# stanfordnlp/mac-network

Measured on AMD Instinct MI355X. Metric: questions/sec fwd+bwd (B=64,d=512,p=12,KB=14x14x1024) at 1/2/4/8 MI355X, higher is better.
Workload: dtype f32 (3xfp16-split emulation); 1 GPU

## Files before the change

include/macx.h:

```cpp
#ifndef MACX_H
#define MACX_H

#include <stddef.h>
#include <stdint.h>

#ifdef __cplusplus
extern "C" {
#endif

#define MACX_ABI_VERSION 5

enum {
  MACX_OK = 0,
  MACX_EINVAL = -1,
  MACX_EUNSUPPORTED = -2,
  MACX_EREJECTED = -3,
  MACX_ESMALL = -4,
  MACX_EWAIT = -5
};

enum { MACX_ACT_NON = 0, MACX_ACT_TANH = 1, MACX_ACT_SIGMOID = 2, MACX_ACT_ELU = 3, MACX_ACT_RELU = 4 };
enum { MACX_INIT_PRM = 0, MACX_INIT_ZERO = 1, MACX_INIT_Q = 2 };
enum { MACX_WRITE_MEM = 0, MACX_WRITE_INFO = 1, MACX_WRITE_SUM = 2, MACX_WRITE_BOTH = 3 };

// ... 241 lines not shown
                       const float* d_kb, const macx_stem_grads*, void* stream);
int macx_stem_forward_w(const macx_stem_shapes*, int act, float keep, uint32_t seed, const macx_stem_params*,
                        const float* images, float* kb, float* saved, size_t saved_floats, const uint32_t* mask_word, void* stream);
int macx_stem_backward_w(const macx_stem_shapes*, int act, float keep, uint32_t seed, const macx_stem_params*,
                         const float* kb, const float* saved, size_t saved_floats, float* ws, size_t ws_floats,
                         const float* d_kb, const macx_stem_grads*, const uint32_t* mask_word, void* stream);

typedef struct macx_conv_shapes { int32_t B, H, W, Cin, Cout, k, stride; } macx_conv_shapes;
size_t macx_conv2d_ws_floats(const macx_conv_shapes*);
int macx_conv2d_fwd(const macx_conv_shapes*, const float* x, const float* w, const float* bias, float* y, void* stream);
int macx_conv2d_bwd_data(const macx_conv_shapes*, const float* dy, const float* w, float* dx, void* stream);
int macx_conv2d_wgrad(const macx_conv_shapes*, const float* x, const float* dy, float* dw, float* ws, size_t ws_floats,
                      void* stream);

int macx_images_to_nhwc(const float* nchw, int B, int C, int HW, float* nhwc, void* stream);

typedef struct macx_enc_shapes { int32_t B, S, V, E, h, b0; } macx_enc_shapes;
typedef struct macx_enc_params { const float* emb; const float* fw_kernel; const float* fw_bias; const float* bw_kernel; const float* bw_bias; } macx_enc_params;
typedef struct macx_enc_grads { float* emb; float* fw_kernel; float* fw_bias; float* bw_kernel; float* bw_bias; } macx_enc_grads;
size_t macx_encoder_saved_floats(const macx_enc_shapes*);
size_t macx_encoder_ws_floats(const macx_enc_shapes*);
int macx_encoder_forward(const macx_enc_shapes*, float keep_input, float keep_question, uint32_t seed, const macx_enc_params*,
                         const int32_t* questions , const int32_t* lengths , float* words ,
                         float* vecQuestions , float* saved, size_t saved_floats, void* stream);
int macx_encoder_backward(const macx_enc_shapes*, float keep_input, float keep_question, uint32_t seed, const macx_enc_params*,
                          const int32_t* questions, const int32_t* lengths, const float* saved, size_t saved_floats,
                          float* ws, size_t ws_floats, const float* d_words, const float* d_vecQuestions,
                          const macx_enc_grads*, void* stream);
int macx_encoder_forward_w(const macx_enc_shapes*, float keep_input, float keep_question, uint32_t seed, const macx_enc_params*,
                           const int32_t* questions , const int32_t* lengths , float* words ,
                           float* vecQuestions , float* saved, size_t saved_floats, const uint32_t* mask_word,
                           void* stream);
int macx_encoder_backward_w(const macx_enc_shapes*, float keep_input, float keep_question, uint32_t seed, const macx_enc_params*,
                            const int32_t* questions, const int32_t* lengths, const float* saved, size_t saved_floats,
                            float* ws, size_t ws_floats, const float* d_words, const float* d_vecQuestions,
                            const macx_enc_grads*, const uint32_t* mask_word, void* stream);

int macx_adam_ema_step(size_t n, float* params, const float* grads, float* m, float* v, float* ema,
                       float lr, float beta1, float beta2, float eps, int step, float clip_norm, float ema_decay,
                       float* ws, float* norm_out, void* stream);
int macx_adam_ema_step_p(size_t n, float* params, const float* grads, float* m, float* v, float* ema,
                         const float* lr_t_dev, float beta1, float beta2, float eps, float clip_norm, float ema_decay,
                         float* ws, float* norm_out, void* stream);
int macx_adam_ema_step_g(size_t n, float* params, const float* grads, float* m, float* v, float* ema,
                         float lr, float beta1, float beta2, float eps, int step, float clip_norm, float ema_decay,
                         float skip_above, uint32_t* guard, float* ws, float* norm_out, void* stream);
int macx_adam_ema_step_pg(size_t n, float* params, const float* grads, float* m, float* v, float* ema,
                          const float* lr_t_dev, float beta1, float beta2, float eps, float clip_norm, float ema_decay,
                          float skip_above, uint32_t* guard, float* ws, float* norm_out, void* stream);

typedef struct macx_gather_entry { const float* src; uint64_t dst_offset; uint64_t count; } macx_gather_entry;
int macx_gather_flat(const macx_gather_entry* table_dev, int entries, float* flat, void* stream);

int macx_kb_gather(const float* kb_images , const int32_t* image_index , int G, int B, int N, int d,
                   float* kb , void* stream);
int macx_kb_gather_bwd(const float* dkb , const int32_t* image_index , int G, int B, int N, int d,
                       float* dkb_images , void* stream);
int macx_kb_gather_l(const float* kb_images , const int32_t* image_index ,
                     const int32_t* image_lengths , int G, int B, int N, int d, float* kb ,
                     int32_t* kb_lengths_out , void* stream);
int macx_kb_gather_bwd_l(const float* dkb , const int32_t* image_index ,
                         const int32_t* image_lengths , int G, int B, int N, int d,
                         float* dkb_images , void* stream);

enum { MACX_FEATURES_F32 = 0, MACX_FEATURES_F16 = 1 };
int macx_features_pack(const float* src, int layout, int n, int C, int HW, void* table, int dtype, size_t row0, size_t rows,
                       int32_t* overflow , void* stream);
int macx_features_gather(const void* table, int dtype, size_t rows, const int32_t* ids , int G, int C, int HW,
                         float* out , void* stream);

int macx_questions_gather(const int32_t* q_words , const int32_t* q_lengths , const int32_t* q_answers ,
                          const int32_t* q_images , const int32_t* q_kb_len ,
                          const float* q_weights , int Q, int S_tab, const int32_t* ids , int B,
                          int S , int32_t* questions , int32_t* lengths , int32_t* answers ,
                          int32_t* image_ids , int32_t* kb_lengths ,
                          float* weights , int32_t* image_index , int G,
                          int32_t* bad , void* stream);
int macx_preds_scatter(const int32_t* pred , const int32_t* ids , int B, int Q, int32_t* table ,
                       void* stream);

int macx_linear(const float* x1, int k1, const float* x2, int k2, int rows,
                const float* W_packed, const float* b, float bias_const, int n_out, int act,
                float* out, void* stream);
#define MACX_PACK_TRANSPOSE 1
#define MACX_PACK_F32MFMA (0 << 1)
#define MACX_PACK_BF16X3 (1 << 1)
#define MACX_PACK_KMAJOR (2 << 1)
int macx_pack_weight(const float* W, int K, int n_out, int flags, float* out, void* stream);
#define MACX_GEMM_NATIVE 0
#define MACX_GEMM_SPLIT 1
#define MACX_GEMM_H2 2
int macx_gemm_mode(int mode);

size_t macx_h2_floats(size_t rows, size_t cols);
int macx_h2_from_f32(const float* src, int B, int N, int C, float* h2, void* stream);
int macx_h2_to_f32(const float* h2, int rows, int C, float* out, void* stream);
int macx_h2_pack_weight(const float* W, int K, int n_out, int transpose, float* out, void* stream);
int macx_h2_gemm_planes(const float* hA, int B, int N, int K, const float* Wh, int n_out, const float* bias, int act, float* hO,
                        void* stream);
int macx_h2_gemm(const float* A, int B, int N, int K, const float* W, int n_out, const float* bias, int act, float* out,
                 float* ws, size_t ws_floats, void* stream);
size_t macx_h2_wgrad_ws_floats(const macx_opts* o, int nt, int R, int Kd, int Jd, int nsplit, int pair);
int macx_h2_wgrad(const macx_opts* o, int nt, int R, int Kd, int Jd, int nsplit, const float* hA, size_t a_stride, int a_shared,
                  const float* hG, size_t g_stride, float* out, const float* hA2, size_t a2_stride, int a2_shared, const float* hG2,
                  size_t g2_stride, float* out2, float* ws, size_t ws_floats, void* stream);
size_t macx_h2_sb_ws_floats(const macx_opts* o, int B, int N, int d, int nsteps, int qpg, int wide);
int macx_h2_sb(const macx_opts* o, int B, int N, int d, int nsteps, int qpg, int wide, const float* hX, size_t x_stride,
               const float* hdI1, size_t g_stride, const float* y, const float* W1a, float* dW1a, float* dW1b, float* dy_part,
               float* ws, size_t ws_floats, void* stream);
int macx_read_chain_time(const macx_opts*, const macx_shapes*, const macx_dropout*, const macx_params*, const macx_inputs*,
                         float* saved, size_t saved_floats, int step, int reps, float* ms_out, void* stream);
int macx_cell_forward_chain_time(const macx_opts*, const macx_shapes*, const macx_dropout*, const macx_params*, const macx_inputs*,
                                 float* saved, size_t saved_floats, float* ws, size_t ws_floats, float* ms_out, void* stream);
int macx_saved_activation(const macx_opts*, const macx_shapes*, int which, int step, const float* saved, size_t saved_floats,
                          float* out, void* stream);
size_t macx_ctrl_inputs_ws_floats(const macx_opts*, const macx_shapes*);
int macx_ctrl_inputs_fwd(const macx_opts*, const macx_shapes*, const macx_params*, const float* vecQuestions, float* ctrl_t,
                         float* ctrl_inputs, float* ws, size_t ws_floats, void* stream);
int macx_ctrl_inputs_bwd(const macx_opts*, const macx_shapes*, const macx_params*, const float* vecQuestions, const float* ctrl_t,
                         const float* d_ctrl_inputs, const macx_param_grads*, float* d_vecQuestions, float* ws, size_t ws_floats,
                         void* stream);
int macx_kb_project(const macx_shapes*, const macx_dropout*, int step, const float* kb,
                    const float* W_packed, const float* b, float* out, float* drop_ws, void* stream);
int macx_control_attend(const macx_shapes*, const float* cc, const float* words, const int32_t* lengths,
                        const float* w, const float* b, float* att, float* control, void* stream);
size_t macx_control_attend_bwd_ws_floats(const macx_shapes*);
int macx_control_attend_bwd(const macx_shapes*, const float* d_control, const float* cc, const float* att, const float* words,
                            const float* w, float* ws, size_t ws_floats, float* d_cc, float* d_words, float* d_w, float* d_b,
                            void* stream);
int macx_dropout_mask(uint32_t seed, uint32_t site, uint32_t step, float keep, uint32_t first,
                      size_t n, float* out, void* stream);
int macx_dropout_mask_w(uint32_t seed, uint32_t site, uint32_t step, float keep, uint32_t first,
                        size_t n, const uint32_t* mask_word, float* out, void* stream);
int macx_wgrad_splits(int M, int Kd, int Jd);
int macx_wgrad(const float* A, int lda, const float* G, int ldg, int M, int Kd, int Jd,
               float* out, float* ws, void* stream);

int macx_answer_loss(const float* logits, const int32_t* answers, int B, int A, float* loss_rows, int32_t* pred,
                     float* dlogits, float grad_scale, void* stream);

enum { MACX_ATT_LOSS_CE = 0, MACX_ATT_LOSS_ENTROPY = 1 };
int macx_att_loss(const float* att, const float* target, const int32_t* lengths, const float* step_weights,
                  const float* row_weights, int p, int B, int n, int kind, int target_steps, float eps, float scale,
                  float* loss_rows, float* d_att, void* stream);

int macx_answer_loss_weighted(const float* logits, const int32_t* answers, const float* weights, int B, int A,
                              float* loss_rows, int32_t* pred, float* dlogits, float* loss_out, double* totals,
                              float grad_scale, void* stream);

int macx_kb_attend_fwd(int B, int N, int d, const float* logits, const float* bias, const float* kb, float* att, float* info,
                       void* stream);
int macx_kb_attend_fwd_l(int B, int N, int d, const float* logits, const float* bias, const float* kb, const int32_t* kb_lengths,
                         float* att, float* info, void* stream);
size_t macx_kb_attend_bwd_ws_floats(int B, int N, int d);
int macx_kb_attend_bwd(int B, int N, int d, const float* att, const float* kb, const float* dinfo, float* dlogits, float* dkb,
                       int accumulate, float* ws, size_t ws_floats, void* stream);

size_t macx_workspace_bytes(const macx_opts*, const macx_shapes*, int for_backward);
int macx_read_fwd(const macx_opts*, const macx_shapes*, const macx_dropout*, const macx_params*, const float* knowledgeBase,
                  const float* memory, const float* control, float* saved, size_t saved_floats, float* info, float* att,
                  void* stream);
int macx_read_fwd_l(const macx_opts*, const macx_shapes*, const macx_dropout*, const macx_params*, const float* knowledgeBase,
                    const int32_t* kb_lengths, const float* memory, const float* control, float* saved, size_t saved_floats,
                    float* info, float* att, void* stream);
int macx_read_bwd(const macx_opts*, const macx_shapes*, const macx_dropout*, const macx_params*, const float* knowledgeBase,
                  const float* saved, size_t saved_floats, float* ws, size_t ws_floats, const float* d_info,
// ... 39 lines not shown
```

mac-network_amd/_lib.py:

```python
import ctypes as C
import os

import torch

from . import build as _build

ABI_VERSION = 5

MACX_OK, MACX_EINVAL, MACX_EUNSUPPORTED, MACX_EREJECTED, MACX_ESMALL, MACX_EWAIT = 0, -1, -2, -3, -4, -5
HANDOFF_BITS = {1: "a chain tile gave up waiting for its step's y", 2: "a filler workgroup gave up waiting for the previous step's write unit"}
STATUS_WORDS = 16
ACT = {"NON": 0, "TANH": 1, "SIGMOID": 2, "ELU": 3, "RELU": 4}
INIT = {"PRM": 0, "ZERO": 1, "Q": 2}
WRITE_INPUTS = {"MEM": 0, "INFO": 1, "SUM": 2, "BOTH": 3}
SEG = {"controls": 0, "memories": 1, "infos": 2, "att_question": 3, "att_kb": 4, "att_self": 5, "att_gate": 6,
       "status": 7}


class MacxOpts(C.Structure):
    _fields_ = [(n, C.c_int32) for n in (
        "abi_version", "init_ctrl", "init_mem", "control_input_unshared", "control_input_act", "control_feed_prev",
        "control_feed_prev_att", "control_feed_inputs", "control_cont_act", "read_mem_act", "read_ctrl_act",
        "write_inputs", "write_self_att", "write_self_att_cont", "write_mem_act", "write_gate", "write_gate_shared")]
    _fields_ += [("write_gate_bias", C.c_float), ("memory_variational_dropout", C.c_int32), ("gemm_family", C.c_int32),
# ... 115 lines not shown
_I, _U, _Z, _F, _V = C.c_int, C.c_uint32, C.c_size_t, C.c_float, C.c_void_p


def _masked(sig):
    restype, a = sig
    return restype, a[:-1] + (_V, a[-1])


_OS = (_P(MacxOpts), _P(MacxShapes))
_RUN = _OS + (_P(MacxDropout), _P(MacxParams), _P(MacxInputs), _V, _Z, _V, _Z)
_BWD = _RUN + (_V, _V, _P(MacxParamGrads), _P(MacxInputGrads))
_UNIT = _OS + (_P(MacxDropout), _P(MacxParams))
_STEM = (_P(MacxStemShapes), _I, _F, _U, _P(MacxStemParams))
_OUT = (_P(MacxOutShapes), _I, _F, _U, _P(MacxOutParams))
_ENC = (_P(MacxEncShapes), _F, _F, _U, _P(MacxEncParams))
_GATHER = (_V, _V, _I, _I, _I, _I, _V, _V)

TABLE = {}
TABLE.update(
    macx_saved_floats=(_Z, _OS + (_I,)),
    macx_ws_floats=(_Z, _OS + (_I,)),
    macx_saved_segment=(_I, _OS + (_I, _I, _P(_Z), _P(_Z))),
    macx_check=(_I, _OS),
    macx_cell_route=(_I, _OS + (_P(MacxDropout), _I, _I, _P(MacxRoute))))
TABLE.update(
    macx_run_status=(_I, _OS + (_I, _V, _Z, _V, _P(_U), _P(C.c_int32))),
    macx_run_status_reset=(_I, _OS + (_I, _V, _Z, _V)),
    macx_handoff_selftest=(_I, (_V, _P(_U))))
TABLE.update(
    macx_cell_begin=(_I, _RUN + (_I, _V)),
    macx_cell_step=(_I, _RUN + (_I, _I, _V)),
    macx_cell_forward=(_I, _RUN + (_I, _V)),
    macx_cell_backward=(_I, _BWD + (_V,)),
    macx_cell_backward_phase=(_I, _BWD + (_I, _V)),
    macx_cell_backward_x=(_I, _BWD + (_P(MacxStateGrads), _V)),
    macx_cell_backward_phase_x=(_I, _BWD + (_P(MacxStateGrads), _I, _V)))
TABLE.update(
    macx_output_saved_floats=(_Z, (_P(MacxOutShapes),)),
    macx_output_ws_floats=(_Z, (_P(MacxOutShapes),)),
    macx_output_forward=(_I, _OUT + (_V, _V, _V, _V, _Z, _V)),
    macx_output_backward=(_I, _OUT + (_V, _V, _V, _Z, _V, _Z, _V, _P(MacxOutGrads), _V, _V, _V)))
TABLE.update(macx_output_forward_w=_masked(TABLE["macx_output_forward"]),
             macx_output_backward_w=_masked(TABLE["macx_output_backward"]))
TABLE.update(
    macx_stem_saved_floats=(_Z, (_P(MacxStemShapes),)),
    macx_stem_ws_floats=(_Z, (_P(MacxStemShapes),)),
    macx_stem_forward=(_I, _STEM + (_V, _V, _V, _Z, _V)),
    macx_stem_backward=(_I, _STEM + (_V, _V, _Z, _V, _Z, _V, _P(MacxStemGrads), _V)))
TABLE.update(macx_stem_forward_w=_masked(TABLE["macx_stem_forward"]),
             macx_stem_backward_w=_masked(TABLE["macx_stem_backward"]))
TABLE.update(
    macx_conv2d_ws_floats=(_Z, (_P(MacxConvShapes),)),
    macx_conv2d_fwd=(_I, (_P(MacxConvShapes), _V, _V, _V, _V, _V)),
    macx_conv2d_bwd_data=(_I, (_P(MacxConvShapes), _V, _V, _V, _V)),
    macx_conv2d_wgrad=(_I, (_P(MacxConvShapes), _V, _V, _V, _V, _Z, _V)),
    macx_images_to_nhwc=(_I, (_V, _I, _I, _I, _V, _V)))
TABLE.update(
    macx_encoder_saved_floats=(_Z, (_P(MacxEncShapes),)),
    macx_encoder_ws_floats=(_Z, (_P(MacxEncShapes),)),
    macx_encoder_forward=(_I, _ENC + (_V, _V, _V, _V, _V, _Z, _V)),
    macx_encoder_backward=(_I, _ENC + (_V, _V, _V, _Z, _V, _Z, _V, _V, _P(MacxEncGrads), _V)))
TABLE.update(macx_encoder_forward_w=_masked(TABLE["macx_encoder_forward"]),
             macx_encoder_backward_w=_masked(TABLE["macx_encoder_backward"]))
TABLE.update(
    macx_adam_ema_step=(_I, (_Z, _V, _V, _V, _V, _V, _F, _F, _F, _F, _I, _F, _F, _V, _V, _V)),
    macx_adam_ema_step_p=(_I, (_Z, _V, _V, _V, _V, _V, _V, _F, _F, _F, _F, _F, _V, _V, _V)),
    macx_adam_ema_step_g=(_I, (_Z, _V, _V, _V, _V, _V, _F, _F, _F, _F, _I, _F, _F, _F, _V, _V, _V, _V)),
    macx_adam_ema_step_pg=(_I, (_Z, _V, _V, _V, _V, _V, _V, _F, _F, _F, _F, _F, _F, _V, _V, _V, _V)))
TABLE.update(macx_gather_flat=(_I, (_V, _I, _V, _V)))
TABLE.update(
    macx_kb_gather=(_I, _GATHER),
    macx_kb_gather_bwd=(_I, _GATHER),
    macx_kb_gather_l=(_I, _GATHER[:2] + (_V,) + _GATHER[2:-1] + (_V, _GATHER[-1])),
    macx_kb_gather_bwd_l=(_I, _GATHER[:2] + (_V,) + _GATHER[2:]))
TABLE.update(
    macx_features_pack=(_I, (_V, _I, _I, _I, _I, _V, _I, _Z, _Z, _V, _V)),
    macx_features_gather=(_I, (_V, _I, _Z, _V, _I, _I, _I, _V, _V)))
FEATURES_DTYPE = {torch.float32: 0, torch.float16: 1}
TABLE.update(
    macx_questions_gather=(_I, (_V,) * 6 + (_I, _I, _V, _I, _I) + (_V,) * 6 + (_V, _I, _V, _V)),
    macx_preds_scatter=(_I, (_V, _V, _I, _I, _V, _V)))
TABLE.update(
    macx_linear=(_I, (_V, _I, _V, _I, _I, _V, _V, _F, _I, _I, _V, _V)),
    macx_pack_weight=(_I, (_V, _I, _I, _I, _V, _V)),
    macx_gemm_mode=(_I, (_I,)))
TABLE.update(
    macx_h2_floats=(_Z, (_Z, _Z)),
    macx_h2_from_f32=(_I, (_V, _I, _I, _I, _V, _V)),
    macx_h2_to_f32=(_I, (_V, _I, _I, _V, _V)),
    macx_h2_pack_weight=(_I, (_V, _I, _I, _I, _V, _V)),
    macx_h2_gemm_planes=(_I, (_V, _I, _I, _I, _V, _I, _V, _I, _V, _V)),
    macx_h2_gemm=(_I, (_V, _I, _I, _I, _V, _I, _V, _I, _V, _V, _Z, _V)),
    macx_h2_wgrad_ws_floats=(_Z, (_P(MacxOpts),) + (_I,) * 6),
    macx_h2_wgrad=(_I, (_P(MacxOpts),) + (_I,) * 5 + (_V, _Z, _I, _V, _Z, _V) * 2 + (_V, _Z, _V)),
    macx_h2_sb_ws_floats=(_Z, (_P(MacxOpts),) + (_I,) * 6),
    macx_h2_sb=(_I, (_P(MacxOpts),) + (_I,) * 6 + (_V, _Z, _V, _Z) + (_V,) * 5 + (_V, _Z, _V)),
    macx_read_chain_time=(_I, _RUN[:7] + (_I, _I, _P(_F), _V)),
    macx_cell_forward_chain_time=(_I, _RUN + (_P(_F), _V)),
    macx_saved_activation=(_I, _OS + (_I, _I, _V, _Z, _V, _V)),
    macx_ctrl_inputs_ws_floats=(_Z, _OS),
    macx_ctrl_inputs_fwd=(_I, _OS + (_P(MacxParams), _V, _V, _V, _V, _Z, _V)),
    macx_ctrl_inputs_bwd=(_I, _OS + (_P(MacxParams), _V, _V, _V, _P(MacxParamGrads), _V, _V, _Z, _V)),
    macx_kb_project=(_I, (_P(MacxShapes), _P(MacxDropout), _I, _V, _V, _V, _V, _V, _V)),
    macx_control_attend=(_I, (_P(MacxShapes),) + (_V,) * 8),
    macx_control_attend_bwd_ws_floats=(_Z, (_P(MacxShapes),)),
    macx_control_attend_bwd=(_I, (_P(MacxShapes),) + (_V,) * 6 + (_Z,) + (_V,) * 5),
    macx_dropout_mask=(_I, (_U, _U, _U, _F, _U, _Z, _V, _V)),
    macx_dropout_mask_w=(_I, (_U, _U, _U, _F, _U, _Z, _V, _V, _V)),
    macx_wgrad_splits=(_I, (_I, _I, _I)),
    macx_wgrad=(_I, (_V, _I, _V, _I, _I, _I, _I, _V, _V, _V)))
TABLE.update(macx_answer_loss=(_I, (_V, _V, _I, _I, _V, _V, _V, _F, _V)))
TABLE.update(macx_att_loss=(_I, (_V,) * 5 + (_I,) * 5 + (_F, _F) + (_V, _V, _V)))
ATT_LOSS_KINDS = {"ce": 0, "entropy": 1}
TABLE.update(macx_answer_loss_weighted=(_I, (_V,) * 3 + (_I, _I) + (_V,) * 5 + (_F, _V)))
TABLE.update(
    macx_kb_attend_fwd=(_I, (_I, _I, _I) + (_V,) * 6),
    macx_kb_attend_fwd_l=(_I, (_I, _I, _I) + (_V,) * 7),
    macx_kb_attend_bwd_ws_floats=(_Z, (_I, _I, _I)),
    macx_kb_attend_bwd=(_I, (_I, _I, _I) + (_V,) * 5 + (_I, _V, _Z, _V)))
TABLE.update(
    macx_workspace_bytes=(_Z, _OS + (_I,)),
    macx_read_fwd=(_I, _UNIT + (_V, _V, _V, _V, _Z, _V, _V, _V)),
    macx_read_fwd_l=(_I, _UNIT + (_V, _V, _V, _V, _V, _Z, _V, _V, _V)),
    macx_read_bwd=(_I, _UNIT + (_V, _V, _Z, _V, _Z, _V, _P(MacxParamGrads), _V, _V, _V, _V)),
    macx_write_fwd=(_I, _UNIT + (_V, _V, _V, _V, _Z, _V, _V)),
    macx_write_bwd=(_I, _UNIT + (_V, _Z, _V, _Z, _V, _P(MacxParamGrads), _V, _V, _V, _V)))
TABLE.update(
    macx_embed_lookup=(_I, (_V, _V, _I, _I, _I, _F, _U, _U, _V, _V)),
    macx_embed_lookup_bwd=(_I, (_V, _V, _I, _I, _I, _I, _F, _U, _U, _V, _V)))
TABLE.update(
    macx_op_act=(_I, (_I, _V, _V, _Z, _I, _V, _V)),
    macx_op_act_bwd=(_I, (_I, _V, _V, _V, _Z, _I, _V, _V, _V)),
    macx_op_binary=(_I, (_I, _I, _V, _V, _Z, _I, _I, _F, _V, _V)),
    macx_op_reduce=(_I, (_I, _V, _Z, _I, _I, _V, _V, _V)),
    macx_op_softmax=(_I, (_V, _V, _I, _Z, _I, _V, _V)),
    macx_op_softmax_bwd=(_I, (_V, _V, _Z, _I, _V, _V)),
    macx_op_dropout=(_I, (_V, _Z, _U, _U, _U, _F, _U, _V, _V)),
    macx_op_dropout_w=(_I, (_V, _Z, _U, _U, _U, _F, _U, _V, _V, _V)))
TABLE.update(
    macx_strerror=(C.c_char_p, (_I,)),
    macx_abi_version=(_I, ()))

EXPORTS = tuple(TABLE)

_lib = None


class MacxError(RuntimeError):
    def __init__(self, code, where):
        self.code = code
        msg = lib().macx_strerror(code).decode() if _lib is not None else str(code)
        super().__init__("%s failed: %s (code %d)" % (where, msg, code))


class HandoffTimeout(RuntimeError):

    def __init__(self, bits, first_step, where="MAC cell run"):
        self.bits, self.first_step = int(bits), int(first_step)
        what = [t for b, t in sorted(HANDOFF_BITS.items()) if self.bits & b] or ["unknown bits"]
        super().__init__("%s: in-launch hand-off timeout (status 0x%x: %s; first at step %d); the run's results are NaN"
                         % (where, self.bits, "; ".join(what), self.first_step))


def lib():
    global _lib
    if _lib is not None:
# ... 34 lines not shown
```

mac-network_amd/csrc/macx_api.hip:

```cpp
#include <hip/hip_runtime.h>
#include <math.h>
#include <stdlib.h>
#include <string.h>

#include "../../include/macx.h"
#include "macx_common.hip.h"
#include "macx_gemm.hip.h"
#include "macx_gemm6.hip.h"
#include "macx_gemm_tn.hip.h"
#include "macx_wgrad6.hip.h"
#include "macx_gemm3h.hip.h"
#include "macx_h2.hip.h"
#include "macx_gemm_h2.hip.h"
#include "macx_chain_api.hip.h"
#include "macx_wgrad_h2.hip.h"
#include "macx_small.hip.h"
#include "macx_ops.hip.h"
#include "macx_conv.hip.h"
#include "macx_kb_gather.hip.h"
#include "macx_features.hip.h"
#include "macx_questions.hip.h"
#include "macx_att_loss.hip.h"

using namespace macx;
// ... 2009 lines not shown
  CKI(unit_check(o, s, false));
  if (!knowledgeBase || !d_info || !d_knowledgeBase || !d_memory || !d_control) return MACX_EINVAL;
  if (!dp || !P || !saved || !ws || !GP) return MACX_EINVAL;
  macx_inputs in{};
  in.knowledgeBase = knowledgeBase;
  macx_input_grads GI{};
  GI.knowledgeBase = d_knowledgeBase;
  CellBwd r(o, s, dp, P, &in, saved, ws, GP, &GI, stream);
  CKI(r.check_bwd_buffers(saved_floats, ws_floats, 0));
  CKI(r.init_state_grads(nullptr, nullptr));
  r.dinfo = StepSlab{d_info, r.d, r.Bd};
  CKI(r.read_unit_bwd(0));
  CKI(r.dy_linear_bwd(0, false));
  CKI(r.read_dc_reduce_all());
  CKI(r.read_linear_wgrads());
  CK(dev_copy(d_memory, r.DM, r.Bd * sizeof(float), r.st));
  CK(dev_copy(d_control, r.DC + r.Bd, r.Bd * sizeof(float), r.st));
  CKI(r.wb.run(r.st));
  CK(r.rs.run(r.st));
  return r.read_weight_contractions();
}

int macx_write_fwd(const macx_opts* o, const macx_shapes* s, const macx_dropout* dp, const macx_params* P,
                   const float* memory, const float* info, const float* control, float* saved, size_t saved_floats,
                   float* new_memory, void* stream) {
  ModeScope ms(o);
  CKI(unit_check(o, s, true));
  if (!dp || !P || !memory || !info || !control || !saved || !new_memory) return MACX_EINVAL;
  if (misaligned(saved)) return MACX_EINVAL;
  const CellRun r(o, s, dp, P, nullptr, saved, 1, stream);
  if (saved_floats < r.L.total) return MACX_ESMALL;
  {
    Packer pk;
    r.add_write_packs(pk);
    if (r.L.bwd_packs) {
      const BwdLayout W = make_bwd(o, s, r.R);
      r.add_write_packs(pk, &W);
    }
    CK(pk.run(r.st));
  }
  CK(dev_copy(r.memories(), memory, r.Bd * sizeof(float), r.st));
  CK(dev_copy(r.info_raw(0), info, r.Bd * sizeof(float), r.st));
  CK(dev_copy(r.controls() + r.Bd, control, r.Bd * sizeof(float), r.st));
  CKI(r.write_step(0, false));
  CK(dev_copy(new_memory, r.memories() + r.Bd, r.Bd * sizeof(float), r.st));
  return MACX_OK;
}

int macx_write_bwd(const macx_opts* o, const macx_shapes* s, const macx_dropout* dp, const macx_params* P,
                   const float* saved, size_t saved_floats, float* ws, size_t ws_floats, const float* d_new_memory,
                   const macx_param_grads* GP, float* d_memory, float* d_info, float* d_control, void* stream) {
  ModeScope ms(o);
  CKI(unit_check(o, s, true));
  if (!d_new_memory || !d_memory || !d_info || !d_control) return MACX_EINVAL;
  if (!dp || !P || !saved || !ws || !GP) return MACX_EINVAL;
  CellBwd r(o, s, dp, P, nullptr, saved, ws, GP, nullptr, stream);
  CKI(r.check_bwd_buffers(saved_floats, ws_floats, 0));
  CKI(r.init_state_grads(d_new_memory, nullptr));
  CKI(r.write_unit_bwd(0));
  const size_t wbytes = (size_t)r.d * sizeof(float);
  CK(dev_copy2d(d_memory, wbytes, ws + r.W.dwin, (size_t)r.win * sizeof(float), wbytes, r.B, r.st));
  if (o->write_gate) CK(axpy(ws + r.W.tmpBd[3], r.Bd, d_memory, r.st));
  CK(dev_copy2d(d_info, wbytes, r.dinfo.base, (size_t)r.dinfo.ld * sizeof(float), wbytes, r.B, r.st));
  CK(dev_copy(d_control, r.DC + r.Bd, r.Bd * sizeof(float), r.st));
  CKI(r.gate_wgrads());
  CKI(r.write_linear_wgrads());
  CKI(r.wb.run(r.st));
  CK(r.rs.run(r.st));
  return MACX_OK;
}

int macx_linear(const float* x1, int k1, const float* x2, int k2, int rows, const float* Wp, const float* b, float bias_const,
                int n_out, int act, float* out, void* stream) {
  if (!x1 || !Wp || !out || rows < 1 || n_out < 16 || n_out % 16) return MACX_EINVAL;
  if (k1 % 16 != 0 || k2 % 16 != 0 || k1 < 16 || (x2 == nullptr) != (k2 == 0)) return MACX_EINVAL;
  if (misaligned(x1) || misaligned(x2) || misaligned(Wp) || misaligned(out)) return MACX_EINVAL;
  LinP l = lin_basic(x1, k1, k1, rows, Wp, b, n_out, act, out, n_out);
  if (x2) { l.seg[1] = LinSeg{x2, k2, k2, 0}; l.Ktot = k1 + k2; }
  l.bias_const = bias_const;
  CK(small_linear_launch(l, 1, (hipStream_t)stream));
  return MACX_OK;
}

int macx_pack_weight(const float* Wt, int K, int n_out, int flags, float* out, void* stream) {
  const int transpose = flags;
  if (!Wt || !out || K < 16 || K % 16 || n_out < 16 || n_out % 16) return MACX_EINVAL;
  const int fmt = transpose >> 1;
  if (fmt < 0 || fmt > 2 || (fmt && K % 32)) return MACX_EINVAL;
  Packer pk;
  if (transpose & 1) pk.add(Wt, 1, K, K, n_out, out, -1, -1, fmt);
  else pk.add(Wt, n_out, 1, K, n_out, out, -1, -1, fmt);
  CK(pk.run((hipStream_t)stream));
  return MACX_OK;
}

int macx_kb_project(const macx_shapes* s, const macx_dropout* dp, int step, const float* kb, const float* Wp, const float* b,
                    float* out, float* bits_ws, void* stream) {
  if (!s || !dp || !kb || !Wp || !b || !out) return MACX_EINVAL;
  if (s->d % 128 != 0 || s->N > K_MAXN || ((size_t)s->B * s->N * s->d) % 32) return MACX_EINVAL;
  hipStream_t st = (hipStream_t)stream;
  const int d = s->d;
  GemmP g;
  memset(&g, 0, sizeof(g));
  g.B = s->B; g.N = s->N; g.K = d; g.Nout = d;
  g.A = kb; g.lda = d;
  g.Wp = Wp; g.out = out; g.ldo = d; g.bias = b; g.act = MACX_ACT_NON;
  if (dp->keep_read < 1.0f) {
    if (!bits_ws) return MACX_EINVAL;
    const size_t n = (size_t)s->B * s->N * d;
    const DropSpec dk = make_drop(dp->keep_read, dp, SITE_READ_KB, step);
    hipLaunchKernelGGL(kb_dropout_kernel, dim3(2048), dim3(256), 0, st, kb, n / 4, dk.key, dk.thr24, dk.inv_keep,
                       (uint32_t)((size_t)s->b0 * s->N * d), bits_ws, reinterpret_cast<uint32_t*>(bits_ws + n), 0u, (uint32_t*)nullptr,
                       dk.word);
    CK(hipGetLastError());
    g.A = bits_ws;
  }
  CK((kb_gemm<A_PLAIN, B_PLAIN, E_BIAS_ACT, false>(g, st)));
  return MACX_OK;
}

int macx_control_attend(const macx_shapes* s, const float* cc, const float* words, const int32_t* lengths, const float* w,
                        const float* b, float* att, float* control, void* stream) {
  if (!s || !cc || !words || !lengths || !w || !b || !att || !control) return MACX_EINVAL;
  if (s->B < 1 || s->S < 1 || s->S > C_MAXS || s->d < 4 || s->d % 4 != 0) return MACX_EINVAL;
  return control_attend(s->B, s->S, s->d, 1, cc, words, lengths, w, b, att, control, (hipStream_t)stream);
}

size_t macx_control_attend_bwd_ws_floats(const macx_shapes* s) {
  if (!s) return 0;
  return al4((size_t)s->B * s->S) + al4((size_t)s->B * s->d) + al4((size_t)s->B);
}

int macx_control_attend_bwd(const macx_shapes* s, const float* d_control, const float* cc, const float* att, const float* words,
                            const float* w, float* ws, size_t ws_floats, float* d_cc, float* d_words, float* d_w, float* d_b,
                            void* stream) {
  if (!s || !d_control || !cc || !att || !words || !w || !ws || !d_cc || !d_words || !d_w || !d_b) return MACX_EINVAL;
  if (s->B < 1 || s->S < 1 || s->S > C_MAXS || s->d < 64 || s->d % 64 != 0) return MACX_EINVAL;
  if (ws_floats < macx_control_attend_bwd_ws_floats(s)) return MACX_ESMALL;
  hipStream_t st = (hipStream_t)stream;
  const int B = s->B, S = s->S, d = s->d;
  float* dw_part = ws + al4((size_t)B * S);
  float* db_part = dw_part + al4((size_t)B * d);
  CKI(control_attend_bwd(B, S, d, 1, d_control, cc, att, words, w, nullptr, ws, d_cc, d_words, 0, dw_part, db_part, st));
  CK(rowsum(dw_part, B, d, d, d_w, st));
  CK(rowsum(db_part, B, 1, 1, d_b, st));
  return MACX_OK;
}

int macx_embed_lookup(const int32_t* ids, const float* emb, int rows, int E, int ld, float keep, uint32_t seed, uint32_t first_row,
                      float* x, void* stream) {
  if (!ids || !emb || !x || rows < 1 || E < 1 || ld < E) return MACX_EINVAL;
  hipLaunchKernelGGL(embed_gather_kernel, dim3(512), dim3(256), 0, (hipStream_t)stream, ids, emb, rows, E, ld, first_row,
                     make_drop(keep, seed, SITE_ENC_INPUT, 0), x);
  CK(hipGetLastError());
  return MACX_OK;
}

int macx_embed_lookup_bwd(const int32_t* ids, const float* dx, int rows, int E, int ld, int V, float keep, uint32_t seed,
                          uint32_t first_row, float* d_emb, void* stream) {
  if (!ids || !dx || !d_emb || rows < 1 || E < 1 || ld < E || V < 1) return MACX_EINVAL;
  hipLaunchKernelGGL(embed_grad_kernel, dim3(V, (E + 1023) / 1024), dim3(256), 0, (hipStream_t)stream, ids, dx, rows, E, ld, first_row,
                     make_drop(keep, seed, SITE_ENC_INPUT, 0), d_emb);
  CK(hipGetLastError());
  return MACX_OK;
}

// ... 1206 lines not shown
```

mac-network_amd/csrc/macx_lin_tile.hip.h:

```cpp
#pragma once
#include "macx_common.hip.h"

namespace macx {

struct LinSeg { const float* x; int ld; int K; size_t zstride; };
struct LinP {
  LinSeg seg[3];
  int Ktot, rows, n_out;
  const float* W; size_t zW;
  const float* bias; size_t zb; float bias_const;
  int act;
  float* out; int ldo; size_t zout;
  const float* actgrad_src; int actgrad_act; int ld_ag; size_t zag;
  int use_drop; DropSpec d1, d2; uint32_t drop_row0;
  int drop_ld;
  float* out_drop; int ld_od;
  const float* addend; int ld_add; size_t zadd;
  const float* part; int part_N; float* part_sum; int part_shift;
};
constexpr int LIN_PART_TILES = 6;

template <int RTL, bool PART = false, bool COH = false, bool COHIN = false, int CTL = 1>
__device__ __forceinline__ void small_linear_tile(const LinP& p, int bx, int by, int z, float (*red)[16 * RTL][20], int tid, bool live = true,
                                                  bool poison = false) {
  constexpr int L_ROWS = 16 * RTL;
  constexpr int NWV = 4;
  static_assert(CTL == 1 || (CTL == 2 && !PART), "one or two column tiles");
  const int lane = tid & 63;
  const int wave = __builtin_amdgcn_readfirstlane(tid >> 6);
  const int c0 = bx * 16 * CTL;
  const int r0 = by * L_ROWS;
  const int li = lane & 15, lg = lane >> 4;

  f32x4 acc[RTL][CTL];
#pragma unroll
  for (int t = 0; t < RTL; ++t)
#pragma unroll
    for (int c = 0; c < CTL; ++c) acc[t][c] = f32x4{0.f, 0.f, 0.f, 0.f};
  int rowc[RTL];
#pragma unroll
  for (int t = 0; t < RTL; ++t) rowc[t] = min(r0 + 16 * t + li, p.rows - 1);

  const float* Wz = p.W + (size_t)z * p.zW + ((size_t)lg * p.n_out + c0 + li) * 4;
  const int nQ = p.Ktot >> 4;
  const int er = tid / (4 * CTL), ecq = (tid % (4 * CTL)) * 4;
  const int erow = min(r0 + er, p.rows - 1), ecol = c0 + ecq;
  f32x4 e_bias = {0.f, 0.f, 0.f, 0.f}, e_add = {0.f, 0.f, 0.f, 0.f}, e_ag = {0.f, 0.f, 0.f, 0.f};
  auto ld4 = [](const float* q) __attribute__((always_inline)) {
    if ((reinterpret_cast<uintptr_t>(q) & 15) == 0) return *reinterpret_cast<const f32x4*>(q);
    return f32x4{q[0], q[1], q[2], q[3]};
  };
  if (er < L_ROWS) {
    if (p.bias) e_bias = ld4(p.bias + (size_t)z * p.zb + ecol);
    if (p.addend) e_add = ld4(p.addend + (size_t)z * p.zadd + (size_t)erow * p.ld_add + ecol);
    if (p.actgrad_src) e_ag = ld4(p.actgrad_src + (size_t)z * p.zag + (size_t)erow * p.ld_ag + ecol);
  }
  constexpr int PF = PART ? 4 : 8;
  const float* pbase[LIN_PART_TILES];
  bool pvalid[LIN_PART_TILES];
  if (PART) {
    const uint32_t first = (uint32_t)rowc[0] * (uint32_t)p.part_N;
    const int t0 = (int)(first >> p.part_shift), t1 = (int)((first + p.part_N - 1) >> p.part_shift);
#pragma unroll
    for (int j = 0; j < LIN_PART_TILES; ++j) {
      const int tt = min(t0 + j, t1);
      const int seg = rowc[0] - (int)(((uint32_t)tt << p.part_shift) / (uint32_t)p.part_N);
      pbase[j] = p.part + ((size_t)tt * 3 + seg) * p.Ktot + lg * 4;
      pvalid[j] = t0 + j <= t1;
    }
  }
  for (int Q0 = wave; Q0 < nQ; Q0 += NWV * PF) {
    f32x4 bf[PF][CTL], af[PF][RTL];
    if (PART) {
      f32x4 pv[PF][LIN_PART_TILES];
#pragma unroll
      for (int u = 0; u < PF; ++u) {
        const int Q = min(Q0 + NWV * u, nQ - 1);
        bf[u][0] = *reinterpret_cast<const f32x4*>(Wz + (size_t)Q * 4 * p.n_out * 4);
#pragma unroll
        for (int j = 0; j < LIN_PART_TILES; ++j) pv[u][j] = *reinterpret_cast<const f32x4*>(pbase[j] + Q * 16);
      }
#pragma unroll
      for (int u = 0; u < PF; ++u) {
        f32x4 sum = pv[u][0];
#pragma unroll
        for (int j = 1; j < LIN_PART_TILES; ++j) sum += pvalid[j] ? pv[u][j] : f32x4{0.f, 0.f, 0.f, 0.f};
        af[u][0] = sum;
        const int Q = Q0 + NWV * u;
        if (live && bx == 0 && Q < nQ && r0 + li < p.rows)
          *reinterpret_cast<f32x4*>(p.part_sum + (size_t)(r0 + li) * p.Ktot + Q * 16 + lg * 4) = sum;
      }
    } else {
#pragma unroll
    for (int u = 0; u < PF; ++u) {
      const int Q = min(Q0 + NWV * u, nQ - 1);
      int s = 0, koff = Q * 16;
      if (koff >= p.seg[0].K) { koff -= p.seg[0].K; s = 1; if (koff >= p.seg[1].K) { koff -= p.seg[1].K; s = 2; } }
      const float* xs = p.seg[s].x + (size_t)z * p.seg[s].zstride + koff + lg * 4;
      const int ld = p.seg[s].ld;
#pragma unroll
      for (int c = 0; c < CTL; ++c) bf[u][c] = *reinterpret_cast<const f32x4*>(Wz + (size_t)Q * 4 * p.n_out * 4 + c * 64);
#pragma unroll
      for (int t = 0; t < RTL; ++t) {
        if constexpr (COHIN) {
          const uint64_t* q8 = reinterpret_cast<const uint64_t*>(xs + (size_t)rowc[t] * ld);
          const uint64_t lo = __hip_atomic_load(q8, __ATOMIC_RELAXED, __HIP_MEMORY_SCOPE_AGENT);
          const uint64_t hi = __hip_atomic_load(q8 + 1, __ATOMIC_RELAXED, __HIP_MEMORY_SCOPE_AGENT);
          af[u][t] = f32x4{__uint_as_float((uint32_t)lo), __uint_as_float((uint32_t)(lo >> 32)), __uint_as_float((uint32_t)hi),
                           __uint_as_float((uint32_t)(hi >> 32))};
          if (poison) { const float nan = __uint_as_float(0x7fc00000u); af[u][t] = f32x4{nan, nan, nan, nan}; }
        } else {
          af[u][t] = *reinterpret_cast<const f32x4*>(xs + (size_t)rowc[t] * ld);
        }
      }
    }
    }
#pragma unroll
    for (int u = 0; u < PF; ++u) {
      if (Q0 + NWV * u < nQ) {
#pragma unroll
        for (int e = 0; e < 4; ++e)
#pragma unroll
          for (int t = 0; t < RTL; ++t)
#pragma unroll
            for (int c = 0; c < CTL; ++c) acc[t][c] = __builtin_amdgcn_mfma_f32_16x16x4f32(af[u][t][e], bf[u][c][e], acc[t][c], 0, 0, 0);
      }
    }
  }
#pragma unroll
  for (int t = 0; t < RTL; ++t)
#pragma unroll
    for (int e = 0; e < 4; ++e)
#pragma unroll
      for (int c = 0; c < CTL; ++c) red[c * NWV + wave][16 * t + lg * 4 + e][li] = acc[t][c][e];
  __syncthreads();
  const int r = tid / (4 * CTL), cqt = (tid % (4 * CTL)) * 4, cs = (cqt >> 4) * NWV, cq = cqt & 15;
  const int row = r0 + r;
  if (live && r < L_ROWS && row < p.rows) {
  f32x4 val, vald = {0.f, 0.f, 0.f, 0.f};
#pragma unroll
  for (int e = 0; e < 4; ++e) {
    float t = ((red[cs][r][cq + e] + red[cs + 1][r][cq + e]) + red[cs + 2][r][cq + e]) + red[cs + 3][r][cq + e];
    val[e] = t;
  }
  const int col = c0 + cqt;
#pragma unroll
  for (int e = 0; e < 4; ++e) {
    float v = val[e];
    v += e_bias[e];
    v += p.bias_const;
    v = act_apply(p.act, v);
    if (p.actgrad_src) v *= act_grad_from_out(p.actgrad_act, e_ag[e]);
    if (p.use_drop) {
      const uint32_t idx = (p.drop_row0 + row) * (uint32_t)(p.drop_ld > 0 ? p.drop_ld : p.n_out) + col + e;
      float f = 1.f;
      if (!keep_bit(idx, run_key(p.d1), p.d1.thr24)) f = 0.f; else f *= p.d1.inv_keep;
      if (!keep_bit(idx, run_key(p.d2), p.d2.thr24)) f = 0.f; else f *= p.d2.inv_keep;
      if (p.use_drop == 2) vald[e] = v * f;
      else v *= f;
    }
    v += e_add[e];
    val[e] = v;
  }
  if (COH) {
    float* o = p.out + (size_t)z * p.zout + (size_t)row * p.ldo + col;
#pragma unroll
    for (int e = 0; e < 4; ++e) __hip_atomic_store(o + e, val[e], __ATOMIC_RELAXED, __HIP_MEMORY_SCOPE_AGENT);
  } else {
    *reinterpret_cast<f32x4*>(p.out + (size_t)z * p.zout + (size_t)row * p.ldo + col) = val;
  }
  if (p.use_drop == 2) {
    if (COH) {
      float* o = p.out_drop + (size_t)row * p.ld_od + col;
#pragma unroll
      for (int e = 0; e < 4; ++e) __hip_atomic_store(o + e, vald[e], __ATOMIC_RELAXED, __HIP_MEMORY_SCOPE_AGENT);
    } else {
      *reinterpret_cast<f32x4*>(p.out_drop + (size_t)row * p.ld_od + col) = vald;
    }
  }
  }
}

}
```

mac-network_amd/csrc/macx_small.hip.h:

```cpp
#pragma once
#include "macx_common.hip.h"
#include "macx_h2.hip.h"
#include "macx_lin_tile.hip.h"

namespace macx {

__global__ void pack_weight_kernel(const float* __restrict__ src, int ld_k, int ld_j, int K, int Nout, float* dst) {
  const size_t total = (size_t)K * Nout;
  for (size_t i = (size_t)blockIdx.x * blockDim.x + threadIdx.x; i < total; i += (size_t)gridDim.x * blockDim.x) {
    const int e = i & 3;
    const size_t t = i >> 2;
    const int j = t % Nout;
    const size_t qg = t / Nout;
    const int g = qg & 3;
    const int Q = qg >> 2;
    const int k = 16 * Q + 4 * g + e;
    dst[i] = src[(size_t)k * ld_k + (size_t)j * ld_j];
  }
}

struct PackDesc { const float* src; float* dst; int ld_k, ld_j, K, Nout; int k_src, n_src; int fmt; int maxabs_n; const float* maxabs; float* exp_dst; float* maxabs_out; };
constexpr int PACK_MAX = 56;
static_assert(sizeof(PackDesc) * PACK_MAX <= 4096, "PackList travels by value as a kernel argument");
struct PackList { PackDesc d[PACK_MAX]; };
// ... 32 lines not shown
      const int j = t % q.Nout;
      const int kt = (int)(t / q.Nout);
      const int k = kt * 32 + kk;
      const float x = (k < q.k_src && j < q.n_src) ? q.src[(size_t)k * q.ld_k + (size_t)j * q.ld_j] : 0.f;
      if (q.fmt == 2) {
        q.dst[i] = x;
      } else {
        const __bf16 h1 = (__bf16)x;
        const float r1 = x - (float)h1;
        const __bf16 h2 = (__bf16)r1;
        const __bf16 h3 = (__bf16)(r1 - (float)h2);
        __bf16* d = reinterpret_cast<__bf16*>(q.dst);
        const size_t plane = (size_t)q.Nout * 32;
        const size_t o = ((size_t)kt * 3 * q.Nout + j) * 32 + kk;
        d[o] = h1; d[o + plane] = h2; d[o + 2 * plane] = h3;
      }
    }
  }
}

__global__ __launch_bounds__(256) void kb_dropout_kernel(const float* __restrict__ kb, size_t n4, uint32_t key, uint32_t thr24,
                                                        float inv_keep, uint32_t first, float* out, uint32_t* bits, uint32_t key2,
                                                        uint32_t* bits2, const uint32_t* word = nullptr) {
  key = run_key(key, word);
  key2 = run_key(key2, word);
  const size_t stride = (size_t)gridDim.x * blockDim.x;
  const size_t n4r = (n4 + 7) & ~(size_t)7;
  for (size_t i = (size_t)blockIdx.x * blockDim.x + threadIdx.x; i < n4r; i += stride) {
    const bool in = i < n4;
    f32x4 v = in ? reinterpret_cast<const f32x4*>(kb)[i] : f32x4{0.f, 0.f, 0.f, 0.f};
    uint32_t nib = 0, nib2 = 0;
#pragma unroll
    for (int e = 0; e < 4; ++e) {
      const uint32_t idx = first + (uint32_t)(i * 4) + e;
      const bool keep = keep_bit(idx, key, thr24);
      nib |= (keep ? 1u : 0u) << e;
      v[e] = keep ? v[e] * inv_keep : 0.f;
      if (bits2) nib2 |= (keep_bit(idx, key2, thr24) ? 1u : 0u) << e;
    }
    if (in) reinterpret_cast<f32x4*>(out)[i] = v;
    uint32_t w = nib << (4 * (threadIdx.x & 7));
    w |= __shfl_xor(w, 1, 64);
    w |= __shfl_xor(w, 2, 64);
    w |= __shfl_xor(w, 4, 64);
    if ((threadIdx.x & 7) == 0 && in) bits[i >> 3] = w;
    if (bits2) {
      uint32_t w2 = nib2 << (4 * (threadIdx.x & 7));
      w2 |= __shfl_xor(w2, 1, 64);
      w2 |= __shfl_xor(w2, 2, 64);
      w2 |= __shfl_xor(w2, 4, 64);
      if ((threadIdx.x & 7) == 0 && in) bits2[i >> 3] = w2;
    }
  }
}

__global__ void mask_bits_kernel(uint32_t key, uint32_t thr24, uint32_t first, size_t nwords, uint32_t* out, const uint32_t* word = nullptr) {
  key = run_key(key, word);
  for (size_t w = (size_t)blockIdx.x * blockDim.x + threadIdx.x; w < nwords; w += (size_t)gridDim.x * blockDim.x) {
    const uint32_t base = first + (uint32_t)(w << 5);
    uint32_t bits = 0;
#pragma unroll
    for (int i = 0; i < 32; ++i) bits |= (keep_bit(base + i, key, thr24) ? 1u : 0u) << i;
    out[w] = bits;
  }
}

__global__ void transpose_kernel(const float* __restrict__ src, int R, int C, float* dst) {
  __shared__ float tile[32][33];
  src += (size_t)blockIdx.z * R * C;
  dst += (size_t)blockIdx.z * R * C;
  const int bx = blockIdx.x * 32, by = blockIdx.y * 32;
  const int tx = threadIdx.x & 31, ty = threadIdx.x >> 5;
  for (int i = ty; i < 32; i += 8) {
    const int r = by + i, c = bx + tx;
    tile[i][tx] = (r < R && c < C) ? src[(size_t)r * C + c] : 0.f;
  }
  __syncthreads();
  for (int i = ty; i < 32; i += 8) {
    const int c = bx + i, r = by + tx;
    if (r < R && c < C) dst[(size_t)c * R + r] = tile[tx][i];
  }
}

template <int RTL, bool PART = false>
__global__ __launch_bounds__(256) void small_linear_kernel(LinP p) {
  __shared__ float red[4][16 * RTL][20];
  small_linear_tile<RTL, PART>(p, blockIdx.x, blockIdx.y, blockIdx.z, red, (int)threadIdx.x);
}

inline hipError_t small_linear_part_launch(const LinP& p, hipStream_t st) {
  if (!p.part || !p.part_sum || p.rows > 128 || p.part_shift < 4 || p.part_shift > 6 ||
      ((p.part_N - 2) >> p.part_shift) + 2 > LIN_PART_TILES) return hipErrorInvalidValue;
  hipLaunchKernelGGL((small_linear_kernel<1, true>), dim3(p.n_out / 16, (p.rows + 15) / 16, 1), dim3(256), 0, st, p);
  return hipGetLastError();
}
inline hipError_t small_linear_launch(const LinP& p, int nz, hipStream_t st) {
  if (p.rows <= 128) {
    hipLaunchKernelGGL(small_linear_kernel<1>, dim3(p.n_out / 16, (p.rows + 15) / 16, nz), dim3(256), 0, st, p);
  } else {
    hipLaunchKernelGGL(small_linear_kernel<4>, dim3(p.n_out / 16, (p.rows + 63) / 64, nz), dim3(256), 0, st, p);
  }
  return hipGetLastError();
}

__global__ void drop2_kernel(const float* __restrict__ x, int rows, int d, uint32_t row0, DropSpec d1, DropSpec d2, float* out, int dl = 0) {
  d1 = drop_resolve(d1);
  d2 = drop_resolve(d2);
  const int n = rows * d;
  if (dl <= 0) dl = d;
  for (int i = blockIdx.x * blockDim.x + threadIdx.x; i < n; i += gridDim.x * blockDim.x) {
    const int r = i / d, j = i - r * d;
    const uint32_t idx = (row0 + (uint32_t)r) * (uint32_t)dl + (uint32_t)j;
    float v = x[i];
    v = drop_apply(v, idx, d1);
    v = drop_apply(v, idx, d2);
    out[i] = v;
  }
}

constexpr int SYNC_WORDS = 64 + 32 * 16;
__global__ void init_states_kernel(int mode_c, const float* __restrict__ prm_c, float* out_c, int mode_m, const float* __restrict__ prm_m,
                                   float* out_m, const float* __restrict__ vecQ, int rows, int d, float* md = nullptr, uint32_t row0 = 0,
                                   DropSpec d1 = DropSpec{}, DropSpec d2 = DropSpec{}, int dl = 0, uint32_t* sync = nullptr) {
  const int n = rows * d;
  if (sync && blockIdx.x == 0)
    for (int i = threadIdx.x; i < SYNC_WORDS; i += blockDim.x) sync[i] = 0u;
  if (md) { d1 = drop_resolve(d1); d2 = drop_resolve(d2); }
  if (dl <= 0) dl = d;
  for (int i = blockIdx.x * blockDim.x + threadIdx.x; i < n; i += gridDim.x * blockDim.x) {
    const float q = (mode_c == 2 || mode_m == 2) ? vecQ[i] : 0.f;
    out_c[i] = mode_c == 0 ? prm_c[i % d] : (mode_c == 2 ? q : 0.f);
    const float m = mode_m == 0 ? prm_m[i % d] : (mode_m == 2 ? q : 0.f);
    out_m[i] = m;
    if (md) {
      const int r = i / d, j = i - r * d;
      const uint32_t idx = (row0 + (uint32_t)r) * (uint32_t)dl + (uint32_t)j;
      md[i] = drop_apply(drop_apply(m, idx, d1), idx, d2);
    }
  }
}

__global__ void bwd_init_kernel(float* DM, size_t slab, int p, const float* __restrict__ d_memory, const float* __restrict__ d_control, int tail,
                                const float* __restrict__ g_mem = nullptr, const float* __restrict__ g_ctrl = nullptr) {
  const size_t per = (size_t)(p + 1) * slab, total = 2 * per + (size_t)tail;
  for (size_t i = (size_t)blockIdx.x * blockDim.x + threadIdx.x; i < total; i += (size_t)gridDim.x * blockDim.x) {
    float v = 0.f;
    if (i < 2 * per) {
      const size_t w = i >= per ? i - per : i;
      if (w >= (size_t)p * slab) {
        const float* src = i >= per ? d_control : d_memory;
        if (src) v = src[w - (size_t)p * slab];
      }
      const float* g = i >= per ? g_ctrl : g_mem;
      if (g) v += g[w];
    }
    DM[i] = v;
  }
}

__global__ void dropout_mask_kernel(uint32_t key, uint32_t thr24, uint32_t first, size_t n, float* out, const uint32_t* word = nullptr) {
  key = run_key(key, word);
  for (size_t i = (size_t)blockIdx.x * blockDim.x + threadIdx.x; i < n; i += (size_t)gridDim.x * blockDim.x)
    out[i] = keep_bit(first + (uint32_t)i, key, thr24) ? 1.f : 0.f;
}

constexpr int ROWSUM_COLS = 16;
__global__ __launch_bounds__(1024) void rowsum_kernel(const float* __restrict__ src, int rows, int n, size_t ld, float* dst, size_t zsrc,
                                                      size_t zdst) {
  __shared__ float red[64][ROWSUM_COLS + 1];
  src += blockIdx.y * zsrc;
  dst += blockIdx.y * zdst;
  const int c = threadIdx.x & (ROWSUM_COLS - 1), rg = threadIdx.x / ROWSUM_COLS;
  const int i = blockIdx.x * ROWSUM_COLS + c;
  float s0 = 0.f, s1 = 0.f;
  if (i < n) {
    int r = rg;
// ... 1078 lines not shown
```

Baseline: 18680 questions/s.

## Split partial-sum linear to 8 rows per workgroup and specialize tile count

```diff
diff --git a/include/macx.h b/include/macx.h
--- a/include/macx.h
+++ b/include/macx.h
@@ -347,6 +347,9 @@
 int macx_linear(const float* x1, int k1, const float* x2, int k2, int rows,
                 const float* W_packed, const float* b, float bias_const, int n_out, int act,
                 float* out, void* stream);
+int macx_linear_part(const float* part, int part_N, int part_shift, int k, int rows,
+                     const float* W_packed, const float* b, float bias_const, int n_out, int act,
+                     float* part_sum, float* out, void* stream);
 #define MACX_PACK_TRANSPOSE 1
 #define MACX_PACK_F32MFMA (0 << 1)
 #define MACX_PACK_BF16X3 (1 << 1)
diff --git a/mac-network_amd/_lib.py b/mac-network_amd/_lib.py
--- a/mac-network_amd/_lib.py
+++ b/mac-network_amd/_lib.py
@@ -221,6 +221,7 @@
     macx_preds_scatter=(_I, (_V, _V, _I, _I, _V, _V)))
 TABLE.update(
     macx_linear=(_I, (_V, _I, _V, _I, _I, _V, _V, _F, _I, _I, _V, _V)),
+    macx_linear_part=(_I, (_V, _I, _I, _I, _I, _V, _V, _F, _I, _I, _V, _V, _V)),
     macx_pack_weight=(_I, (_V, _I, _I, _I, _V, _V)),
     macx_gemm_mode=(_I, (_I,)))
 TABLE.update(
diff --git a/mac-network_amd/csrc/macx_api.hip b/mac-network_amd/csrc/macx_api.hip
--- a/mac-network_amd/csrc/macx_api.hip
+++ b/mac-network_amd/csrc/macx_api.hip
@@ -2115,6 +2115,19 @@
   return MACX_OK;
 }
 
+int macx_linear_part(const float* part, int part_N, int part_shift, int k, int rows, const float* Wp, const float* b, float bias_const,
+                     int n_out, int act, float* part_sum, float* out, void* stream) {
+  if (!part || !Wp || !part_sum || !out || rows < 1 || rows > 128 || n_out < 16 || n_out % 16 || k < 16 || k % 16) return MACX_EINVAL;
+  if (part_N < 1 || part_shift < 4 || part_shift > 6 || ((part_N - 2) >> part_shift) + 2 > LIN_PART_TILES) return MACX_EINVAL;
+  if ((1 << part_shift) > 2 * part_N) return MACX_EINVAL;
+  if (misaligned(part) || misaligned(Wp) || misaligned(part_sum) || misaligned(out)) return MACX_EINVAL;
+  LinP l = lin_basic(part_sum, k, k, rows, Wp, b, n_out, act, out, n_out);
+  l.bias_const = bias_const;
+  l.part = part; l.part_N = part_N; l.part_sum = part_sum; l.part_shift = part_shift;
+  CK(small_linear_part_launch(l, (hipStream_t)stream));
+  return MACX_OK;
+}
+
 int macx_pack_weight(const float* Wt, int K, int n_out, int flags, float* out, void* stream) {
   const int transpose = flags;
   if (!Wt || !out || K < 16 || K % 16 || n_out < 16 || n_out % 16) return MACX_EINVAL;
diff --git a/mac-network_amd/csrc/macx_lin_tile.hip.h b/mac-network_amd/csrc/macx_lin_tile.hip.h
--- a/mac-network_amd/csrc/macx_lin_tile.hip.h
+++ b/mac-network_amd/csrc/macx_lin_tile.hip.h
@@ -20,17 +20,21 @@
 };
 constexpr int LIN_PART_TILES = 6;
 
-template <int RTL, bool PART = false, bool COH = false, bool COHIN = false, int CTL = 1>
+constexpr int LIN_PART_ROWS = 8;
+template <int RTL, bool PART = false, bool COH = false, bool COHIN = false, int CTL = 1, int NPT = LIN_PART_TILES>
 __device__ __forceinline__ void small_linear_tile(const LinP& p, int bx, int by, int z, float (*red)[16 * RTL][20], int tid, bool live = true,
                                                   bool poison = false) {
   constexpr int L_ROWS = 16 * RTL;
   constexpr int NWV = 4;
   static_assert(CTL == 1 || (CTL == 2 && !PART), "one or two column tiles");
+  static_assert(!PART || (RTL == 1 && NPT >= 1 && NPT <= LIN_PART_TILES), "PART: 8 questions per workgroup, 1 .. LIN_PART_TILES tiles each");
+  constexpr int RL = PART ? LIN_PART_ROWS : L_ROWS;
   const int lane = tid & 63;
   const int wave = __builtin_amdgcn_readfirstlane(tid >> 6);
   const int c0 = bx * 16 * CTL;
-  const int r0 = by * L_ROWS;
+  const int r0 = by * RL;
   const int li = lane & 15, lg = lane >> 4;
+  const int lr = PART ? li & (RL - 1) : li, lh = PART ? li >> 3 : 0;
 
   f32x4 acc[RTL][CTL];
 #pragma unroll
@@ -39,7 +43,7 @@
     for (int c = 0; c < CTL; ++c) acc[t][c] = f32x4{0.f, 0.f, 0.f, 0.f};
   int rowc[RTL];
 #pragma unroll
-  for (int t = 0; t < RTL; ++t) rowc[t] = min(r0 + 16 * t + li, p.rows - 1);
+  for (int t = 0; t < RTL; ++t) rowc[t] = min(r0 + 16 * t + lr, p.rows - 1);
 
   const float* Wz = p.W + (size_t)z * p.zW + ((size_t)lg * p.n_out + c0 + li) * 4;
   const int nQ = p.Ktot >> 4;
@@ -50,21 +54,22 @@
     if ((reinterpret_cast<uintptr_t>(q) & 15) == 0) return *reinterpret_cast<const f32x4*>(q);
     return f32x4{q[0], q[1], q[2], q[3]};
   };
-  if (er < L_ROWS) {
+  if (er < RL) {
     if (p.bias) e_bias = ld4(p.bias + (size_t)z * p.zb + ecol);
     if (p.addend) e_add = ld4(p.addend + (size_t)z * p.zadd + (size_t)erow * p.ld_add + ecol);
     if (p.actgrad_src) e_ag = ld4(p.actgrad_src + (size_t)z * p.zag + (size_t)erow * p.ld_ag + ecol);
   }
-  constexpr int PF = PART ? 4 : 8;
-  const float* pbase[LIN_PART_TILES];
-  bool pvalid[LIN_PART_TILES];
+  constexpr int PF = 8;
+  const float* pbase[NPT];
+  bool pvalid[NPT];
   if (PART) {
     const uint32_t first = (uint32_t)rowc[0] * (uint32_t)p.part_N;
     const int t0 = (int)(first >> p.part_shift), t1 = (int)((first + p.part_N - 1) >> p.part_shift);
+    const int seg0 = rowc[0] - (int)(((uint32_t)t0 << p.part_shift) / (uint32_t)p.part_N);
 #pragma unroll
-    for (int j = 0; j < LIN_PART_TILES; ++j) {
+    for (int j = 0; j < NPT; ++j) {
       const int tt = min(t0 + j, t1);
-      const int seg = rowc[0] - (int)(((uint32_t)tt << p.part_shift) / (uint32_t)p.part_N);
+      const int seg = tt == t0 ? seg0 : 0;
       pbase[j] = p.part + ((size_t)tt * 3 + seg) * p.Ktot + lg * 4;
       pvalid[j] = t0 + j <= t1;
     }
@@ -72,23 +77,31 @@
   for (int Q0 = wave; Q0 < nQ; Q0 += NWV * PF) {
     f32x4 bf[PF][CTL], af[PF][RTL];
     if (PART) {
-      f32x4 pv[PF][LIN_PART_TILES];
+      f32x4 pv[PF / 2][NPT];
 #pragma unroll
-      for (int u = 0; u < PF; ++u) {
-        const int Q = min(Q0 + NWV * u, nQ - 1);
-        bf[u][0] = *reinterpret_cast<const f32x4*>(Wz + (size_t)Q * 4 * p.n_out * 4);
+      for (int v = 0; v < PF / 2; ++v) {
 #pragma unroll
-        for (int j = 0; j < LIN_PART_TILES; ++j) pv[u][j] = *reinterpret_cast<const f32x4*>(pbase[j] + Q * 16);
+        for (int h = 0; h < 2; ++h)
+          bf[2 * v + h][0] = *reinterpret_cast<const f32x4*>(Wz + (size_t)min(Q0 + NWV * (2 * v + h), nQ - 1) * 4 * p.n_out * 4);
+        const int Q = min(Q0 + NWV * (2 * v + lh), nQ - 1);
+#pragma unroll
+        for (int j = 0; j < NPT; ++j) pv[v][j] = *reinterpret_cast<const f32x4*>(pbase[j] + Q * 16);
       }
 #pragma unroll
-      for (int u = 0; u < PF; ++u) {
-        f32x4 sum = pv[u][0];
+      for (int v = 0; v < PF / 2; ++v) {
+        f32x4 sum = pv[v][0];
 #pragma unroll
-        for (int j = 1; j < LIN_PART_TILES; ++j) sum += pvalid[j] ? pv[u][j] : f32x4{0.f, 0.f, 0.f, 0.f};
-        af[u][0] = sum;
-        const int Q = Q0 + NWV * u;
-        if (live && bx == 0 && Q < nQ && r0 + li < p.rows)
-          *reinterpret_cast<f32x4*>(p.part_sum + (size_t)(r0 + li) * p.Ktot + Q * 16 + lg * 4) = sum;
+        for (int j = 1; j < NPT; ++j) sum += pvalid[j] ? pv[v][j] : f32x4{0.f, 0.f, 0.f, 0.f};
+        if (NPT < LIN_PART_TILES) sum += f32x4{0.f, 0.f, 0.f, 0.f};
+        const int Q = Q0 + NWV * (2 * v + lh);
+        if (live && bx == 0 && Q < nQ && r0 + lr < p.rows)
+          *reinterpret_cast<f32x4*>(p.part_sum + (size_t)(r0 + lr) * p.Ktot + Q * 16 + lg * 4) = sum;
+        af[2 * v][0] = sum;
+#pragma unroll
+        for (int e = 0; e < 4; ++e) {
+          const float se = sum[e];
+          af[2 * v + 1][0][e] = __builtin_bit_cast(float, __builtin_amdgcn_update_dpp(0, __builtin_bit_cast(int, se), 0x128, 0xF, 0xF, false));
+        }
       }
     } else {
 #pragma unroll
@@ -136,7 +149,7 @@
   __syncthreads();
   const int r = tid / (4 * CTL), cqt = (tid % (4 * CTL)) * 4, cs = (cqt >> 4) * NWV, cq = cqt & 15;
   const int row = r0 + r;
-  if (live && r < L_ROWS && row < p.rows) {
+  if (live && r < RL && row < p.rows) {
   f32x4 val, vald = {0.f, 0.f, 0.f, 0.f};
 #pragma unroll
   for (int e = 0; e < 4; ++e) {
diff --git a/mac-network_amd/csrc/macx_small.hip.h b/mac-network_amd/csrc/macx_small.hip.h
--- a/mac-network_amd/csrc/macx_small.hip.h
+++ b/mac-network_amd/csrc/macx_small.hip.h
@@ -138,16 +138,28 @@
   }
 }
 
-template <int RTL, bool PART = false>
+template <int RTL, bool PART = false, int NPT = LIN_PART_TILES>
 __global__ __launch_bounds__(256) void small_linear_kernel(LinP p) {
   __shared__ float red[4][16 * RTL][20];
-  small_linear_tile<RTL, PART>(p, blockIdx.x, blockIdx.y, blockIdx.z, red, (int)threadIdx.x);
-}
-
+  small_linear_tile<RTL, PART, false, false, 1, NPT>(p, blockIdx.x, blockIdx.y, blockIdx.z, red, (int)threadIdx.x);
+}
+
+template <int NPT>
+inline void small_linear_part_launch_as(const LinP& p, hipStream_t st) {
+  hipLaunchKernelGGL((small_linear_kernel<1, true, NPT>), dim3(p.n_out / 16, (p.rows + LIN_PART_ROWS - 1) / LIN_PART_ROWS, 1), dim3(256), 0, st, p);
+}
 inline hipError_t small_linear_part_launch(const LinP& p, hipStream_t st) {
-  if (!p.part || !p.part_sum || p.rows > 128 || p.part_shift < 4 || p.part_shift > 6 ||
+  if (!p.part || !p.part_sum || p.rows > 128 || p.part_N < 1 || p.part_shift < 4 || p.part_shift > 6 ||
       ((p.part_N - 2) >> p.part_shift) + 2 > LIN_PART_TILES) return hipErrorInvalidValue;
-  hipLaunchKernelGGL((small_linear_kernel<1, true>), dim3(p.n_out / 16, (p.rows + 15) / 16, 1), dim3(256), 0, st, p);
+  const int T = 1 << p.part_shift, g = std::min(T, p.part_N & -p.part_N);
+  const int npt = ((T - g + p.part_N - 1) >> p.part_shift) + 1;
+  switch (npt) {
+    case 1: case 2: small_linear_part_launch_as<2>(p, st); break;
+    case 3: small_linear_part_launch_as<3>(p, st); break;
+    case 4: small_linear_part_launch_as<4>(p, st); break;
+    case 5: small_linear_part_launch_as<5>(p, st); break;
+    default: small_linear_part_launch_as<LIN_PART_TILES>(p, st); break;
+  }
   return hipGetLastError();
 }
 inline hipError_t small_linear_launch(const LinP& p, int nz, hipStream_t st) {
```

New measurement: 18960 questions/s (median of 6 runs). +1.5%, better.
